# Electron-Labs/eth-lc-plonky2

Hardware: AMD Instinct MI355X
Metric: lc_proofs_per_hour (higher is better)
Workload: dtype u64

## Files before the change

### eth-lc-plonky2_amd/csrc/witness_rows.hip

```cpp
#include <cstring>
#include "internal.hpp"
#include "row_stage.hpp"
#include "sha_layout.hpp"
#include "sha_rows.hpp"
#include "pos_rows.hpp"
#include "prover_kernels.hpp"
#include "u32_rows.hpp"
#include "rec_rows.hpp"
#include "pos_plan.hpp"
#include "u32_plan.hpp"

using namespace lcp2;

namespace lcp2 {
int scratch_ensure(lcp2_ctx *ctx, int slot, size_t bytes, void **out) {
  if (ctx->scratch_bytes[slot] < bytes) {
    if (ctx->scratch[slot]) { LCP2_HIP(ctx, hipStreamSynchronize(ctx->stream)); LCP2_HIP(ctx, hipFree(ctx->scratch[slot])); ctx->scratch[slot] = nullptr; ctx->scratch_bytes[slot] = 0; }
    const size_t want = bytes + bytes / 4 + 4096;
    LCP2_HIP(ctx, hipMalloc(&ctx->scratch[slot], want));
    ctx->scratch_bytes[slot] = want;
  }
  *out = ctx->scratch[slot];
  return LCP2_OK;
}
}

namespace {
constexpr size_t ENDS_OK = ~(size_t)0;
size_t ends_problem(const uint32_t *ends, size_t count, size_t total) {
  if (!total) return ENDS_OK;
  for (size_t l = 0; l < count; l++)
    if (ends[l] < (l ? ends[l - 1] : 0) || ends[l] > total) return l;
  return count && ends[count - 1] == total ? ENDS_OK : count;
}
}

static_assert(sizeof(lcp2_sha_job) == sizeof(ShaJobDev) && sizeof(lcp2_cell) == sizeof(CellDev), "ABI structs must match the kernels'");

extern "C" int lcp2_sha256_witness(lcp2_ctx *ctx, const lcp2_sha_job *jobs, size_t njobs, const uint32_t *level_start, uint32_t nlevels,
                                   const uint32_t *words_in, size_t nwords, uint64_t *wires, uint64_t n, uint32_t *digests) {
  if (!ctx || !wires || (njobs && (!jobs || !level_start || nlevels == 0)) || (nwords && !words_in)) return LCP2_E_INVALID;
  if (njobs == 0) return LCP2_OK;
  if (const ShaProblem refused = sha_jobs_problem((const ShaJobDev *)jobs, njobs, level_start, nlevels, nwords, n); refused.problem)
    return ctx->fail(LCP2_E_INVALID, sha_problem_str(refused.problem));
  LCP2_HIP(ctx, hipSetDevice(ctx->device));
  void *d_jobs, *d_words, *d_rec;
  LCP2_TRY(scratch_ensure(ctx, 0, njobs * sizeof(lcp2_sha_job), &d_jobs));
  LCP2_TRY(scratch_ensure(ctx, 1, std::max<size_t>(nwords, 1) * 4, &d_words));
  LCP2_TRY(scratch_ensure(ctx, 2, njobs * (size_t)SHA_REC_WORDS * 4, &d_rec));
  Stage stage{ctx};
  LCP2_TRY(stage.behind(d_jobs, jobs, njobs * sizeof(lcp2_sha_job)));
  if (nwords) LCP2_TRY(stage.behind(d_words, words_in, nwords * 4));
  {
    ProfScope ps(ctx, LCP2_K_SHA256, 96.0 * njobs + 8.0 * 108 * SHA_ROWS * njobs);
    for (uint32_t l = 0; l < nlevels; l++)
      launch_sha_jobs_level(ctx->stream, (const ShaJobDev *)d_jobs, level_start[l], level_start[l + 1] - level_start[l],
                            (const uint32_t *)d_words, (uint32_t *)d_rec);
    launch_sha_fill_rows(ctx->stream, (const ShaJobDev *)d_jobs, (u32)njobs, (const uint32_t *)d_rec, (u64 *)wires, n);
  }
  LCP2_HIP(ctx, hipGetLastError());
  char *back = digests ? stage.room(njobs * 32) : nullptr;
  if (digests)
    LCP2_HIP(ctx, hipMemcpy2DAsync(back ? (void *)back : (void *)digests, 32, (const uint32_t *)d_rec + SHA_REC_DIGEST,
                                   (size_t)SHA_REC_WORDS * 4, 32, njobs, hipMemcpyDeviceToHost, ctx->stream));
  LCP2_HIP(ctx, hipStreamSynchronize(ctx->stream));
  if (back) memcpy(digests, back, njobs * 32);
  return LCP2_OK;
}

extern "C" int lcp2_scatter_cells(lcp2_ctx *ctx, const lcp2_cell *cells, size_t ncells, uint64_t *wires, uint64_t n) {
  if (!ctx || !wires || (ncells && !cells)) return LCP2_E_INVALID;
  if (!ncells) return LCP2_OK;
  if (scatter_cells_problem((const CellDev *)cells, ncells, n) != ncells) return ctx->fail(LCP2_E_INVALID, "scatter: row out of range");
  LCP2_HIP(ctx, hipSetDevice(ctx->device));
  void *d;
  LCP2_TRY(scratch_ensure(ctx, 3, ncells * sizeof(lcp2_cell), &d));
  LCP2_TRY(Stage{ctx}.behind(d, cells, ncells * sizeof(lcp2_cell)));
  launch_scatter_cells(ctx->stream, (const CellDev *)d, ncells, (u64 *)wires, n);
  LCP2_HIP(ctx, hipGetLastError());
  LCP2_HIP(ctx, hipStreamSynchronize(ctx->stream));
  return LCP2_OK;
}

extern "C" int lcp2_poseidon_gate_rows(lcp2_ctx *ctx, const lcp2_poseidon_row *rows, size_t nrows, uint64_t *wires, uint64_t n) {
  static_assert(sizeof(lcp2_poseidon_row) == sizeof(PoseidonRowDev), "row job layouts must agree");
  if (!ctx || !wires || (nrows && !rows)) return LCP2_E_INVALID;
  if (!nrows) return LCP2_OK;
  for (size_t i = 0; i < nrows; i++)
    if (pos_row_problem(((const PoseidonRowDev *)rows)[i], n)) return ctx->fail(LCP2_E_INVALID, "poseidon rows: row out of range or swap flag not boolean");
  LCP2_HIP(ctx, hipSetDevice(ctx->device));
  void *d;
  LCP2_TRY(scratch_ensure(ctx, 0, nrows * sizeof(lcp2_poseidon_row), &d));
  LCP2_TRY(Stage{ctx}.behind(d, rows, nrows * sizeof(lcp2_poseidon_row)));
  launch_poseidon_gate_rows(ctx->stream, (const PoseidonRowDev *)d, nrows, (u64 *)wires, n, ctx->d_rc);
  LCP2_HIP(ctx, hipGetLastError());
  LCP2_HIP(ctx, hipStreamSynchronize(ctx->stream));
  return LCP2_OK;
}

extern "C" int lcp2_u32_gate_rows(lcp2_ctx *ctx, const lcp2_u32_job *jobs, size_t njobs, lcp2_mem jobs_mem, uint64_t *wires, uint64_t n) {
  static_assert(sizeof(lcp2_u32_job) == 24 && sizeof(lcp2_u32_job) == sizeof(U32JobDev), "job layouts must agree");
  static_assert(LCP2_U32_ARITHMETIC == U32_KIND_ARITHMETIC && LCP2_U32_ADD_MANY == U32_KIND_ADD_MANY && LCP2_U32_SUBTRACTION == U32_KIND_SUBTRACTION &&
                LCP2_U32_RANGE_CHECK == U32_KIND_RANGE_CHECK && LCP2_U32_COMPARISON == U32_KIND_COMPARISON, "kind numbering must agree");
  if (!ctx || !wires || (njobs && !jobs)) return LCP2_E_INVALID;
  if (jobs_mem != LCP2_MEM_HOST && jobs_mem != LCP2_MEM_DEVICE) return ctx->fail(LCP2_E_INVALID, "u32 rows: bad lcp2_mem");
  if (!njobs) return LCP2_OK;
  const U32JobDev *list = (const U32JobDev *)jobs;
  if (jobs_mem == LCP2_MEM_HOST)
    for (size_t i = 0; i < njobs; i++)
      if (u32 problem = u32_job_problem(list[i], n))
        return ctx->fail(LCP2_E_INVALID, "u32 rows: job " + std::to_string(i) + ": " + u32_problem_str(problem));
  LCP2_HIP(ctx, hipSetDevice(ctx->device));
  RefusalFlag flag{ctx};
  LCP2_TRY(flag.begin());
  if (jobs_mem == LCP2_MEM_DEVICE) {
    launch_u32_gate_rows(ctx->stream, list, njobs, (u64 *)wires, n, flag.d);
  } else {
    constexpr size_t PIECE = (size_t)1 << 20;
    void *d;
    LCP2_TRY(scratch_ensure(ctx, 0, std::min(njobs, PIECE) * sizeof(lcp2_u32_job), &d));
    for (size_t at = 0; at < njobs; at += PIECE) {
      const size_t count = std::min(PIECE, njobs - at);
      LCP2_TRY(Stage{ctx}.behind(d, list + at, count * sizeof(lcp2_u32_job), njobs <= PIECE));
      launch_u32_gate_rows(ctx->stream, (const U32JobDev *)d, count, (u64 *)wires, n, flag.d);
    }
  }
  return flag.end("u32 rows", u32_problem_str, "the valid jobs are written");
}

namespace {
// ... 121 lines not shown
```

### eth-lc-plonky2_amd/host/builder.cpp

```cpp
#include <cstdio>
#include <algorithm>
#include <atomic>
#include <chrono>
#include <cstdlib>
#include <map>
#include <thread>
#include "host_internal.hpp"

namespace lc {

const uint32_t SHA_K[64] = {
    0x428a2f98, 0x71374491, 0xb5c0fbcf, 0xe9b5dba5, 0x3956c25b, 0x59f111f1, 0x923f82a4, 0xab1c5ed5, 0xd807aa98, 0x12835b01,
    0x243185be, 0x550c7dc3, 0x72be5d74, 0x80deb1fe, 0x9bdc06a7, 0xc19bf174, 0xe49b69c1, 0xefbe4786, 0x0fc19dc6, 0x240ca1cc,
    0x2de92c6f, 0x4a7484aa, 0x5cb0a9dc, 0x76f988da, 0x983e5152, 0xa831c66d, 0xb00327c8, 0xbf597fc7, 0xc6e00bf3, 0xd5a79147,
    0x06ca6351, 0x14292967, 0x27b70a85, 0x2e1b2138, 0x4d2c6dfc, 0x53380d13, 0x650a7354, 0x766a0abb, 0x81c2c92e, 0x92722c85,
    0xa2bfe8a1, 0xa81a664b, 0xc24b8b70, 0xc76c51a3, 0xd192e819, 0xd6990624, 0xf40e3585, 0x106aa070, 0x19a4c116, 0x1e376c08,
    0x2748774c, 0x34b0bcb5, 0x391c0cb3, 0x4ed8aa4a, 0x5b9cca4f, 0x682e6ff3, 0x748f82ee, 0x78a5636f, 0x84c87814, 0x8cc70208,
    0x90befffa, 0xa4506ceb, 0xbef9a3f7, 0xc67178f2};
const uint32_t SHA_IV[8] = {0x6a09e667, 0xbb67ae85, 0x3c6ef372, 0xa54ff53a, 0x510e527f, 0x9b05688c, 0x1f83d9ab, 0x5be0cd19};

static inline uint32_t rotr(uint32_t x, int r) { return (x >> r) | (x << (32 - r)); }

void PartialWitness::set_target(Target t, F value) { entries_.push_back({t.id, value % GOLDILOCKS_P}); }
void PartialWitness::set_hash256_target(const Hash256Target &t, const uint8_t v[32]) {
// ... 550 lines not shown
    case Op::SHA: break;
  }
}

void CircuitData::generate_witness(const PartialWitness &pw, std::vector<uint64_t> &wires, std::vector<F> &public_inputs) const {
  const Impl *d = impl_.get();
  const uint64_t n = 1ull << desc_.params.degree_bits;
  wires.assign((size_t)desc_.params.num_wires * n, 0);
  Values V(d);
  for (auto &e : pw.entries()) V.set(e.first, e.second, "PartialWitness");
  std::vector<lcp2_cell> raw;
  std::vector<const Op *> pending;
  for (const Op &op : d->ops) pending.push_back(&op);
  while (!pending.empty()) {
    std::vector<const Op *> waiting;
    for (const Op *opp : pending) {
      const Op &op = *opp;
      if (!host_op_ready(op, V)) { waiting.push_back(opp); continue; }
      if (op.kind == Op::SHA) eval_sha(op, V, wires, n);
      else host_op_eval(op, V, raw);
    }
    if (waiting.size() == pending.size()) throw UnsatisfiedError("a generator is waiting for a target that is never set");
    pending.swap(waiting);
  }
  for (const lcp2_cell &c : raw) wires[(size_t)c.col * n + c.row] = c.value;
  for (const CellBinding &c : d->cells) wires[(size_t)c.col * n + c.row] = V.get(c.var, "wire cell");
  public_inputs.clear();
  for (uint32_t v : d->public_inputs) public_inputs.push_back(V.get(v, "public input"));
}

CircuitData::~CircuitData() {
  if (impl_) {
    if (impl_->cell_buf_pinned) lcp2_host_unregister(impl_->ctx, impl_->cell_buf.data());
    if (impl_->d_wires) lcp2_buffer_free(impl_->ctx, impl_->d_wires);
    if (impl_->gpu) lcp2_circuit_destroy(impl_->gpu);
    if (impl_->verifier) lcp2_circuit_destroy(impl_->verifier);
  }
}

void CircuitData::verifier_only_data(uint64_t digest[4], std::vector<uint64_t> &cap) const {
  if (!impl_->gpu) throw std::runtime_error("verifier_only_data needs attach_gpu()");
  cap.assign((size_t)4 << desc_.params.cap_height, 0);
  if (lcp2_circuit_digest(impl_->gpu, digest, cap.data()) != LCP2_OK) throw std::runtime_error("lcp2_circuit_digest failed");
}

void CircuitData::attach_gpu(lcp2_ctx *ctx) {
  lcp2_circuit_desc cd = desc_.c_desc();
  int rc;
  if (impl_->compact) {
    lcp2_circuit_rows rows{};
    rows.gate_of_row = impl_->gate_of_row.data(); rows.num_rows = impl_->nrows; rows.pad_gate = G_NOOP;
    rows.row_constants = impl_->compact_consts.data();
    rows.bindings = impl_->compact_bindings.data(); rows.num_bindings = impl_->compact_bindings.size(); rows.bindings_mem = LCP2_MEM_HOST;
    rows.num_classes = (uint32_t)impl_->parent.size();
    cd.constants_sigmas = nullptr;
    rc = lcp2_circuit_create_from_rows(ctx, &cd, &rows, &impl_->gpu);
  } else {
    rc = lcp2_circuit_create(ctx, &cd, &impl_->gpu);
  }
  if (rc != LCP2_OK) throw std::runtime_error(std::string("lcp2_circuit_create: ") + lcp2_status_str(rc) + " (" + lcp2_last_error(ctx) + ")");
  impl_->ctx = ctx;
  const size_t bytes = (size_t)desc_.params.num_wires * ((size_t)1 << desc_.params.degree_bits) * 8;
  if (lcp2_buffer_alloc(ctx, bytes, &impl_->d_wires) != LCP2_OK || lcp2_buffer_zero(ctx, impl_->d_wires, bytes) != LCP2_OK)
    throw std::runtime_error(std::string("witness buffer: ") + lcp2_last_error(ctx));
}

// ... 77 lines not shown
          if (backoff < 8) backoff++;
          continue;
        }
        idle.fetch_add(1, std::memory_order_acq_rel);
        while (!stop.load(std::memory_order_acquire) && epoch.load(std::memory_order_acquire) == e0) {
          if (idle.load(std::memory_order_acquire) >= active.load(std::memory_order_acquire)) stop.store(true, std::memory_order_release);
          else std::this_thread::yield();
        }
        idle.fetch_sub(1, std::memory_order_acq_rel);
      }
    } catch (...) {
      failure[k] = std::current_exception();
      stop.store(true, std::memory_order_release);
    }
    active.fetch_sub(1, std::memory_order_acq_rel);
  };
  std::vector<std::thread> threads;
  for (unsigned k = 1; k < K; k++) threads.emplace_back(lane_main, k);
  lane_main(0);
  for (auto &t : threads) t.join();
  for (unsigned k = 0; k < K; k++) if (failure[k]) std::rethrow_exception(failure[k]);
  host_ops.clear();
  for (unsigned k = 0; k < K; k++) {
    host_ops.insert(host_ops.end(), mine[k].begin(), mine[k].end());
    cells.insert(cells.end(), lane_cells[k].begin(), lane_cells[k].end());
    pos_rows.insert(pos_rows.end(), lane_rows[k].begin(), lane_rows[k].end());
  }
  std::sort(host_ops.begin(), host_ops.end());
}

void CircuitData::generate_witness_gpu(const PartialWitness &pw, std::vector<F> &public_inputs) {
  Impl *d = impl_.get();
  if (!d->gpu) throw std::runtime_error("generate_witness_gpu needs attach_gpu()");
  const uint64_t n = 1ull << desc_.params.degree_bits;
  Values V(d);
  for (auto &e : pw.entries()) V.set(e.first, e.second, "PartialWitness");
  std::vector<const Op *> host_ops, sha_ops;
  for (const Op &op : d->ops) (op.kind == Op::SHA ? sha_ops : host_ops).push_back(&op);
  std::vector<lcp2_cell> cells;
  std::vector<lcp2_poseidon_row> pos_rows;
  const bool prof = getenv("LCP2_PROF") != nullptr;
  auto now = [] { return std::chrono::steady_clock::now(); };
  auto ms = [](std::chrono::steady_clock::time_point a, std::chrono::steady_clock::time_point b) { return std::chrono::duration<double, std::milli>(b - a).count(); };
  double t_host = 0;
  if (d->host_lanes.lane_of_op.size() != d->ops.size()) {
    unsigned want = 1;
    if (const char *e = getenv("LCP2_HOST_LANES")) want = (unsigned)atoi(e);
    d->host_lanes = plan_host_lanes(d, std::max(1u, std::min(want, 8u)));
  }
  HostPhaseStats st;
  bool recording = !d->gpu_plan.ready;
  GpuWitnessPlan recorded;
  size_t n_batches = 0;
  const auto t_begin = now();
  while (true) {
    const auto t0 = now();
    run_host_phase(d, d->host_lanes, host_ops, V, cells, pos_rows, st);
    t_host += ms(t0, now());
    if (sha_ops.empty()) break;
    const size_t batch_no = n_batches++;
    if (d->gpu_plan.ready && batch_no < d->gpu_plan.batches.size()) {
      const ShaBatchPlan &B = d->gpu_plan.batches[batch_no];
      bool applies = B.ops_left.size() < sha_ops.size();
      std::vector<uint32_t> words(B.word_vars.size());
      for (size_t k = 0; k < words.size() && applies; k++) {
        if (!V.known(B.word_vars[k])) applies = false;
        else words[k] = as_u32(V.val[B.word_vars[k]], "sha256 message word");
      }
      if (applies) {
        std::vector<uint32_t> digests(B.jobs.size() * 8);
        int rc = lcp2_sha256_witness(d->ctx, B.jobs.data(), B.jobs.size(), B.level_start.data(), (uint32_t)B.level_start.size() - 1, words.data(), words.size(),
                                     (uint64_t *)d->d_wires, n, digests.data());
        if (rc != LCP2_OK) throw std::runtime_error(std::string("lcp2_sha256_witness: ") + lcp2_status_str(rc) + " (" + lcp2_last_error(d->ctx) + ")");
        for (size_t k = 0; k < B.jobs.size(); k++)
          for (int w = 0; w < 8; w++) V.set(B.out[k][w], digests[k * 8 + w], "sha256 digest");
        sha_ops.clear();
        for (uint32_t k : B.ops_left) sha_ops.push_back(&d->ops[k]);
        continue;
      }
      d->gpu_plan = GpuWitnessPlan();
      recording = false;
    }
    std::map<uint32_t, uint32_t> produced;
    std::vector<lcp2_sha_job> jobs;
    std::vector<uint32_t> level, words, word_vars;
    std::vector<const Op *> batch, later;
    for (const Op *op : sha_ops) {
      lcp2_sha_job job{};
      job.first_row = op->first_row;
      uint32_t lvl = 0;
      bool ok = true;
      size_t words_mark = words.size();
      for (int i = 0; i < 16 && ok; i++) {
// ... 17 lines not shown
    for (uint32_t l : level) level_start[l + 1]++;
    for (uint32_t l = 0; l < nlev; l++) level_start[l + 1] += level_start[l];
    {
      std::vector<uint32_t> fill(level_start.begin(), level_start.end() - 1);
      for (uint32_t s = 0; s < jobs.size(); s++) { newslot[s] = fill[level[s]]++; order[newslot[s]] = s; }
    }
    std::vector<lcp2_sha_job> sorted(jobs.size());
    for (uint32_t s = 0; s < jobs.size(); s++) {
      lcp2_sha_job j = jobs[s];
      for (int i = 0; i < 16; i++)
        if (j.in_src[i] < 0) { uint32_t ref = (uint32_t)~j.in_src[i]; j.in_src[i] = ~(int32_t)(newslot[ref >> 3] * 8 + (ref & 7)); }
      sorted[newslot[s]] = j;
    }
    std::vector<uint32_t> digests(jobs.size() * 8);
    int rc = lcp2_sha256_witness(d->ctx, sorted.data(), sorted.size(), level_start.data(), nlev, words.data(), words.size(),
                                 (uint64_t *)d->d_wires, n, digests.data());
    if (rc != LCP2_OK) throw std::runtime_error(std::string("lcp2_sha256_witness: ") + lcp2_status_str(rc) + " (" + lcp2_last_error(d->ctx) + ")");
    for (uint32_t s = 0; s < batch.size(); s++)
      for (int w = 0; w < 8; w++) V.set(batch[s]->out8[w], digests[(size_t)newslot[s] * 8 + w], "sha256 digest");
    if (recording) {
      ShaBatchPlan B;
      B.jobs = sorted; B.word_vars = word_vars; B.level_start = level_start;
      for (const Op *op : later) B.ops_left.push_back((uint32_t)(op - d->ops.data()));
      B.out.resize(jobs.size());
      for (uint32_t s = 0; s < batch.size(); s++)
        for (int w = 0; w < 8; w++) B.out[newslot[s]][w] = d->find(batch[s]->out8[w]);
      recorded.batches.push_back(std::move(B));
    }
    sha_ops.swap(later);
  }
  if (!host_ops.empty()) throw UnsatisfiedError("a generator is waiting for a target that is never set");
  const auto t_rows = now();
  int rc = lcp2_poseidon_gate_rows(d->ctx, pos_rows.data(), pos_rows.size(), (uint64_t *)d->d_wires, n);
  if (rc != LCP2_OK) throw std::runtime_error(std::string("lcp2_poseidon_gate_rows: ") + lcp2_status_str(rc) + " (" + lcp2_last_error(d->ctx) + ")");
  if (!d->gpu_plan.ready) {
    GpuWitnessPlan fresh;
    std::vector<bool> listed(d->fill_copies ? d->parent.size() : 0, false);
    for (const CellBinding &c : d->cells) {
      uint32_t g = d->gate_of_row[c.row];
      if (g == G_SHA_ADD || g == G_SHA_ROUND_A || g == G_SHA_ROUND_E || g == G_SHA_SCHED || g == G_POSEIDON) continue;
      const uint32_t root = d->find(c.var);
      if (d->fill_copies) {
        if (listed[root]) continue;
        listed[root] = true;
      }
      fresh.host_cells.push_back(CellBinding{c.row, c.col, root});
    }
    if (recording) { fresh.batches = std::move(recorded.batches); fresh.ready = true; }
    d->gpu_plan = std::move(fresh);
  }
  std::vector<lcp2_cell> &buf = d->cell_buf;
  if (buf.size() != d->gpu_plan.host_cells.size()) {
    if (d->cell_buf_pinned) { lcp2_host_unregister(d->ctx, buf.data()); d->cell_buf_pinned = false; }
    buf.resize(d->gpu_plan.host_cells.size());
    for (size_t k = 0; k < buf.size(); k++) { buf[k].row = d->gpu_plan.host_cells[k].row; buf[k].col = d->gpu_plan.host_cells[k].col; }
    if (!buf.empty()) d->cell_buf_pinned = lcp2_host_register(d->ctx, buf.data(), buf.size() * sizeof(lcp2_cell)) == LCP2_OK;
  }
  for (size_t k = 0; k < buf.size(); k++) {
    const uint32_t var = d->gpu_plan.host_cells[k].var;
    if (!V.known(var)) throw UnsatisfiedError("target has no value: wire cell");
    buf[k].value = V.val[var];
  }
  const auto t_scatter = now();
  d->cells_sent = buf.size() + cells.size();
  if (d->fill_copies) {
    rc = lcp2_witness_fill_copies(d->gpu, buf.data(), buf.size(), LCP2_MEM_HOST, (uint64_t *)d->d_wires, nullptr);
    if (rc == LCP2_OK) rc = lcp2_witness_fill_copies(d->gpu, cells.data(), cells.size(), LCP2_MEM_HOST, (uint64_t *)d->d_wires, nullptr);
    if (rc != LCP2_OK) throw std::runtime_error(std::string("lcp2_witness_fill_copies: ") + lcp2_status_str(rc) + " (" + lcp2_last_error(d->ctx) + ")");
  } else {
    rc = lcp2_scatter_cells(d->ctx, buf.data(), buf.size(), (uint64_t *)d->d_wires, n);
    if (rc == LCP2_OK) rc = lcp2_scatter_cells(d->ctx, cells.data(), cells.size(), (uint64_t *)d->d_wires, n);
    if (rc != LCP2_OK) throw std::runtime_error(std::string("lcp2_scatter_cells: ") + lcp2_status_str(rc));
  }
  if (prof)
    printf("  witness generation %.2f ms: host generators %.2f ms on %u lane(s) (%zu sweeps, %zu visits of %zu ops, %zu PoseidonGate rows), SHA-256 batches %.2f ms, "
           "PoseidonGate rows on the device + cell list %.2f ms, scatter of %zu cells %.2f ms\n",
           ms(t_begin, now()), t_host, d->host_lanes.lanes, st.sweeps, st.visits, d->ops.size(), pos_rows.size(), ms(t_begin, t_rows) - t_host, ms(t_rows, t_scatter), cells.size() + buf.size(), ms(t_scatter, now()));
  public_inputs.clear();
  for (uint32_t v : d->public_inputs) public_inputs.push_back(V.get(v, "public input"));
}

void CircuitData::set_fill_copies(bool on) {
  if (impl_->fill_copies == on) return;
  impl_->fill_copies = on;
  impl_->gpu_plan = GpuWitnessPlan();
}
size_t CircuitData::cells_sent_last() const { return impl_->cells_sent; }

void CircuitData::read_device_witness(std::vector<uint64_t> &wires) const {
  const size_t words = (size_t)desc_.params.num_wires << desc_.params.degree_bits;
  wires.resize(words);
  if (!impl_->d_wires || lcp2_buffer_read(impl_->ctx, wires.data(), impl_->d_wires, words * 8) != LCP2_OK)
    throw std::runtime_error("read_device_witness failed");
}

ProofWithPublicInputs CircuitData::prove(const PartialWitness &pw) {
  if (!impl_->gpu) throw std::runtime_error("CircuitData::prove needs attach_gpu(): there is no CPU prover in this library");
  ProofWithPublicInputs out;
  generate_witness_gpu(pw, out.public_inputs);
  out.proof.assign(lcp2_proof_words(&desc_.params), 0);
  int rc = lcp2_prove(impl_->gpu, (const uint64_t *)impl_->d_wires, LCP2_MEM_DEVICE, out.public_inputs.data(), out.public_inputs.size(),
                      out.proof.data(), out.proof.size());
  if (rc == LCP2_E_UNSAT) throw UnsatisfiedError(std::string("lcp2_prove: ") + lcp2_last_error(impl_->ctx));
  if (rc != LCP2_OK) throw std::runtime_error(std::string("lcp2_prove: ") + lcp2_status_str(rc) + " (" + lcp2_last_error(impl_->ctx) + ")");
  return out;
}

std::string CircuitData::describe_report(const lcp2_witness_report &r) const {
  if (r.gate_violations == 0 && r.copy_violations == 0) return "the witness satisfies every gate and copy constraint";
  auto cell = [](uint64_t row, uint32_t wire) { return "(" + std::to_string(row) + ", " + std::to_string(wire) + ")"; };
  std::string text;
  if (r.gate_violations) {
    const char *name = r.gate_index < desc_.gates.size() && r.gate_index < G_COUNT ? gate_name(r.gate_index) : "gate ?";
    text = "row " + std::to_string(r.gate_row) + ", gate " + name + ", constraint " + std::to_string(r.gate_constraint) + " (" +
           std::to_string(r.gate_violations) + " gate constraints violated)";
  }
  if (r.copy_violations) {
    if (!text.empty()) text += "; ";
    text += "copy constraint " + cell(r.copy_row, r.copy_wire) + " != " +
            (r.copy_to_wire == 0xFFFFFFFFu ? std::string("(no cell: the sigma value is no cell id)") : cell(r.copy_to_row, r.copy_to_wire)) + " (" +
// ... 66 lines not shown
```

### eth-lc-plonky2_amd/host/host_internal.hpp

```cpp
#pragma once
#include <algorithm>
#include <cstring>
#include <functional>
#include "lc_plonky2.hpp"
#include "../csrc/pos_rows.hpp"

namespace lc {

constexpr int SHA_ADD_OPS = 3;
constexpr uint32_t ARITH_OPS = 20;
constexpr uint32_t SHA_ROWS_PER_HASH = 48 + 128 + 3 + 128 + 3;

struct GateSetLayout {
  std::vector<std::pair<uint32_t, uint32_t>> groups;
  uint32_t num_selectors = 0, num_regs = 1;
  std::vector<lcp2_gate> gates;
  std::vector<uint32_t> code;
  std::vector<uint64_t> imm;
};
GateSetLayout build_gate_set(uint32_t max_degree);

using lcp2::POS_WIRE_INPUT; using lcp2::POS_WIRE_OUTPUT; using lcp2::POS_WIRE_SWAP; using lcp2::POS_WIRE_DELTA; using lcp2::POS_WIRE_PARTIAL;
using lcp2::POS_GATE_WIRES; using lcp2::pos_wire_full_sbox_0; using lcp2::pos_wire_full_sbox_1;
const uint64_t *poseidon_round_constants();
// ... 18 lines not shown

extern const uint32_t SHA_K[64];
extern const uint32_t SHA_IV[8];

struct Op {
  enum Kind { CONST, ARITH, SHA, BITS, POSEIDON, INV, EXT_INV, SPLIT32, HINT } kind;
  uint32_t out = 0, x = 0, y = 0, z = 0;
  F c0 = 0, c1 = 0;
  std::array<uint32_t, 16> in{};
  std::array<uint32_t, 8> out8{};
  uint32_t first_row = 0;
  std::vector<uint32_t> hint_in;
  std::function<void(const std::vector<F> &, std::vector<F> &)> hint_fn;
  std::vector<uint32_t> internal;
};

struct CellBinding { uint32_t row, col, var; };
struct HostLanes {
  std::vector<uint8_t> lane_of_op;
  unsigned lanes = 1;
};

struct ShaBatchPlan {
  std::vector<lcp2_sha_job> jobs;
  std::vector<uint32_t> word_vars;
  std::vector<uint32_t> level_start;
  std::vector<std::array<uint32_t, 8>> out;
  std::vector<uint32_t> ops_left;
};
struct GpuWitnessPlan {
  bool ready = false;
  std::vector<ShaBatchPlan> batches;
  std::vector<CellBinding> host_cells;
};

struct CircuitData::Impl {
  CircuitConfig config;
  uint32_t nrows = 0;
  std::vector<uint32_t> gate_of_row;
  std::vector<std::array<F, 2>> row_consts;
  std::vector<CellBinding> cells;
  std::vector<uint32_t> parent;
  std::vector<Op> ops;
  std::vector<uint32_t> public_inputs;
  lcp2_ctx *ctx = nullptr;
  void *d_wires = nullptr;
  lcp2_circuit *gpu = nullptr;
  lcp2_circuit *verifier = nullptr;
  HostLanes host_lanes;
  GpuWitnessPlan gpu_plan;
  std::vector<lcp2_cell> cell_buf;
  bool cell_buf_pinned = false;
  bool compact = false;
  std::vector<uint64_t> compact_consts;
  std::vector<lcp2_copy_binding> compact_bindings;
  std::vector<std::pair<uint32_t, uint32_t>> selector_groups;
  BuildTimes times;
  bool fill_copies = false;
  size_t cells_sent = 0;
  mutable std::vector<F> value_store;
  mutable std::vector<uint32_t> stamp_store;
  mutable uint32_t epoch = 0;
  uint32_t find(uint32_t v) const { while (parent[v] != v) v = parent[v]; return v; }
};

void expand_constants_sigmas(const CircuitData::Impl *d, CircuitDescription &D, BuildTimes *times);

}
```

### eth-lc-plonky2_amd/host/lc_plonky2.hpp

```cpp
#pragma once
#include <array>
#include <cstdint>
#include <functional>
#include <map>
#include <memory>
#include <stdexcept>
#include <string>
#include <vector>
#include "../../include/lcp2.h"

namespace lc {

using F = uint64_t;
constexpr F GOLDILOCKS_P = 0xFFFFFFFF00000001ull;

struct Target { uint32_t id = 0xFFFFFFFFu; };
struct BoolTarget { Target target; };
struct U32Target { Target t; };
using Hash256Target = std::array<U32Target, 8>;

struct UnsatisfiedError : std::runtime_error { using std::runtime_error::runtime_error; };
struct VerifyError : std::runtime_error { using std::runtime_error::runtime_error; };

struct CircuitConfig {
// ... 88 lines not shown
};

struct BuildTimes { double gadgets_ms = 0, matrix_ms = 0, identity_ms = 0, classes_ms = 0, cycles_ms = 0; };

struct CircuitDescription {
  lcp2_params params{};
  std::vector<uint64_t> constants_sigmas;
  std::vector<uint64_t> k_is;
  uint32_t num_selectors = 0;
  std::vector<lcp2_gate> gates;
  std::vector<uint32_t> code;
  std::vector<uint64_t> imm;
  uint32_t num_public_inputs = 0, num_regs = 1;
  lcp2_circuit_desc c_desc() const;
};

class CircuitData {
 public:
  ~CircuitData();
  const CircuitDescription &description() const { return desc_; }
  const CircuitDescription &expanded_description() const;
  BuildTimes build_times() const;
  size_t build_upload_bytes() const;
  uint32_t degree_bits() const { return desc_.params.degree_bits; }
  uint32_t quotient_degree_factor() const { return desc_.params.quotient_degree_factor; }
  void generate_witness(const PartialWitness &pw, std::vector<uint64_t> &wires, std::vector<F> &public_inputs) const;
  void attach_gpu(lcp2_ctx *ctx);
  void verifier_only_data(uint64_t digest[4], std::vector<uint64_t> &constants_sigmas_cap) const;
  ProofWithPublicInputs prove(const PartialWitness &pw);
  void generate_witness_gpu(const PartialWitness &pw, std::vector<F> &public_inputs);
  void read_device_witness(std::vector<uint64_t> &wires) const;
  void set_fill_copies(bool on);
  size_t cells_sent_last() const;
  std::string diagnose(const PartialWitness &pw);
  std::string diagnose_witness(const std::vector<uint64_t> &wires, const std::vector<F> &public_inputs) const;
  std::string describe_report(const lcp2_witness_report &report) const;
  void verify(const ProofWithPublicInputs &proof) const;
  bool verify_batch(const uint64_t *proofs, size_t count, const uint64_t *public_inputs, int32_t *failed_checks) const;
  struct Impl;
  const Impl *impl_for_tools() const { return impl_.get(); }

 private:
  friend class CircuitBuilder;
  CircuitData() = default;
  mutable CircuitDescription desc_;
  std::unique_ptr<Impl> impl_;
};

}
```

### include/lcp2.h

```cpp
#ifndef LCP2_H
#define LCP2_H
#include <stddef.h>
#include <stdint.h>

#ifdef __cplusplus
extern "C" {
#endif

#define LCP2_ABI_VERSION 2

typedef enum {
  LCP2_OK = 0,
  LCP2_E_INVALID = -1,
  LCP2_E_NODEVICE = -2,
  LCP2_E_HIP = -3,
  LCP2_E_OOM = -4,
  LCP2_E_UNSAT = -5,
  LCP2_E_UNSUPPORTED = -6,
  LCP2_E_VERIFY = -7
} lcp2_status;

typedef enum { LCP2_MEM_HOST = 0, LCP2_MEM_DEVICE = 1 } lcp2_mem;

#define LCP2_MAX_FRI_LAYERS 8
// ... 46 lines not shown
  LCP2_FIELD_SHL = 16
};
int lcp2_field_op_batch(lcp2_ctx *ctx, const uint64_t *a, const uint64_t *b, uint64_t *out, size_t count, uint32_t op, lcp2_mem mem);

int lcp2_merkle_cap(lcp2_ctx *ctx, const uint64_t *leaves, size_t nleaves, size_t leaf_len,
                    uint32_t cap_height, lcp2_mem mem, uint64_t *cap );

int lcp2_ntt_batch(lcp2_ctx *ctx, uint64_t *data, size_t ncols, uint32_t log_n, int inverse,
                   uint64_t shift, lcp2_mem mem);

int lcp2_lde_batch(lcp2_ctx *ctx, const uint64_t *coeffs, uint64_t *out, size_t ncols, uint32_t log_n,
                   uint32_t rate_bits, lcp2_mem mem);

int lcp2_sha256_tree(lcp2_ctx *ctx, const uint8_t *leaves, uint32_t height, size_t trees,
                     uint8_t *nodes, uint32_t *round_trace, lcp2_mem mem);

typedef struct {
  uint32_t first_row;
  int32_t in_src[16];
} lcp2_sha_job;
typedef struct {
  uint32_t row, col;
  uint64_t value;
} lcp2_cell;
int lcp2_sha256_witness(lcp2_ctx *ctx, const lcp2_sha_job *jobs, size_t njobs, const uint32_t *level_start, uint32_t nlevels,
                        const uint32_t *words_in, size_t nwords, uint64_t *wires, uint64_t n, uint32_t *digests);
int lcp2_scatter_cells(lcp2_ctx *ctx, const lcp2_cell *cells, size_t ncells, uint64_t *wires, uint64_t n);
typedef struct {
  uint32_t row;
  uint32_t swap;
  uint64_t in[12];
} lcp2_poseidon_row;
int lcp2_poseidon_gate_rows(lcp2_ctx *ctx, const lcp2_poseidon_row *rows, size_t nrows, uint64_t *wires, uint64_t n);
enum { LCP2_U32_ARITHMETIC = 0, LCP2_U32_ADD_MANY = 1, LCP2_U32_SUBTRACTION = 2, LCP2_U32_RANGE_CHECK = 3, LCP2_U32_COMPARISON = 4 };
typedef struct {
  uint32_t row;
  uint16_t kind;
  uint16_t op;
  uint32_t in[4];
} lcp2_u32_job;
int lcp2_u32_gate_rows(lcp2_ctx *ctx, const lcp2_u32_job *jobs, size_t njobs, lcp2_mem jobs_mem,
                       uint64_t *wires , uint64_t n);

enum { LCP2_REC_ARITHMETIC = 0, LCP2_REC_BASE_SUM, LCP2_REC_ARITHMETIC_EXT, LCP2_REC_MUL_EXT, LCP2_REC_REDUCING,
       LCP2_REC_REDUCING_EXT, LCP2_REC_POSEIDON_MDS, LCP2_REC_RANDOM_ACCESS, LCP2_REC_EXPONENTIATION,
       LCP2_REC_COSET_INTERPOLATION, LCP2_REC_KINDS };
enum { LCP2_REC_IMM = 0, LCP2_REC_CELL = 1 };
typedef struct {
  uint64_t v;
  uint32_t col;
  uint32_t src;
} lcp2_rec_operand;
typedef struct {
  uint32_t row;
  uint16_t kind;
  uint16_t op;
  uint32_t first_operand, reserved;
} lcp2_rec_job;
int lcp2_rec_gate_rows(lcp2_ctx *ctx, const lcp2_rec_job *jobs, size_t njobs,
                       const lcp2_rec_operand *operands, size_t noperands,
                       const uint32_t *level_ends , size_t nlevels,
                       lcp2_mem lists_mem ,
                       uint64_t *wires , uint32_t ncols, uint64_t n);

enum { LCP2_PLAN_IMM = 0, LCP2_PLAN_CELL = 1, LCP2_PLAN_PREV = 2 };
typedef struct { uint32_t row, first_operand; } lcp2_pos_job;
// ... 224 lines not shown
```

Before: 9196.

## Replay recorded witness plan with async enqueues and a single stream wait

Adds non-blocking enqueue variants of the SHA-256, Poseidon-row and scatter entry points, and a replay path for witness generation once a single-batch plan has been recorded. The replay launches the SHA-256 kernels before running the host generators, so host work overlaps device work, then enqueues the rows and cells and waits on the stream only once. Digest-dependent generators and late cells are handled afterwards. Pinned host buffers for words and digests let the copies run asynchronously. The risk is added complexity and a fallback to the recording path whenever replay preconditions fail.

```diff
diff --git a/eth-lc-plonky2_amd/csrc/witness_rows.hip b/eth-lc-plonky2_amd/csrc/witness_rows.hip
--- a/eth-lc-plonky2_amd/csrc/witness_rows.hip
+++ b/eth-lc-plonky2_amd/csrc/witness_rows.hip
@@ -37,8 +37,9 @@
 
 static_assert(sizeof(lcp2_sha_job) == sizeof(ShaJobDev) && sizeof(lcp2_cell) == sizeof(CellDev), "ABI structs must match the kernels'");
 
-extern "C" int lcp2_sha256_witness(lcp2_ctx *ctx, const lcp2_sha_job *jobs, size_t njobs, const uint32_t *level_start, uint32_t nlevels,
-                                   const uint32_t *words_in, size_t nwords, uint64_t *wires, uint64_t n, uint32_t *digests) {
+namespace {
+int sha256_witness(lcp2_ctx *ctx, const lcp2_sha_job *jobs, size_t njobs, const uint32_t *level_start, uint32_t nlevels,
+                   const uint32_t *words_in, size_t nwords, uint64_t *wires, uint64_t n, uint32_t *digests, bool wait) {
   if (!ctx || !wires || (njobs && (!jobs || !level_start || nlevels == 0)) || (nwords && !words_in)) return LCP2_E_INVALID;
   if (njobs == 0) return LCP2_OK;
   if (const ShaProblem refused = sha_jobs_problem((const ShaJobDev *)jobs, njobs, level_start, nlevels, nwords, n); refused.problem)
@@ -49,8 +50,8 @@
   LCP2_TRY(scratch_ensure(ctx, 1, std::max<size_t>(nwords, 1) * 4, &d_words));
   LCP2_TRY(scratch_ensure(ctx, 2, njobs * (size_t)SHA_REC_WORDS * 4, &d_rec));
   Stage stage{ctx};
-  LCP2_TRY(stage.behind(d_jobs, jobs, njobs * sizeof(lcp2_sha_job)));
-  if (nwords) LCP2_TRY(stage.behind(d_words, words_in, nwords * 4));
+  LCP2_TRY(stage.behind(d_jobs, jobs, njobs * sizeof(lcp2_sha_job), wait));
+  if (nwords) LCP2_TRY(stage.behind(d_words, words_in, nwords * 4, wait));
   {
     ProfScope ps(ctx, LCP2_K_SHA256, 96.0 * njobs + 8.0 * 108 * SHA_ROWS * njobs);
     for (uint32_t l = 0; l < nlevels; l++)
@@ -59,30 +60,31 @@
     launch_sha_fill_rows(ctx->stream, (const ShaJobDev *)d_jobs, (u32)njobs, (const uint32_t *)d_rec, (u64 *)wires, n);
   }
   LCP2_HIP(ctx, hipGetLastError());
-  char *back = digests ? stage.room(njobs * 32) : nullptr;
+  char *back = digests && wait ? stage.room(njobs * 32) : nullptr;
   if (digests)
     LCP2_HIP(ctx, hipMemcpy2DAsync(back ? (void *)back : (void *)digests, 32, (const uint32_t *)d_rec + SHA_REC_DIGEST,
                                    (size_t)SHA_REC_WORDS * 4, 32, njobs, hipMemcpyDeviceToHost, ctx->stream));
+  if (!wait) return LCP2_OK;
   LCP2_HIP(ctx, hipStreamSynchronize(ctx->stream));
   if (back) memcpy(digests, back, njobs * 32);
   return LCP2_OK;
 }
 
-extern "C" int lcp2_scatter_cells(lcp2_ctx *ctx, const lcp2_cell *cells, size_t ncells, uint64_t *wires, uint64_t n) {
+int scatter_cells(lcp2_ctx *ctx, const lcp2_cell *cells, size_t ncells, uint64_t *wires, uint64_t n, bool wait) {
   if (!ctx || !wires || (ncells && !cells)) return LCP2_E_INVALID;
   if (!ncells) return LCP2_OK;
   if (scatter_cells_problem((const CellDev *)cells, ncells, n) != ncells) return ctx->fail(LCP2_E_INVALID, "scatter: row out of range");
   LCP2_HIP(ctx, hipSetDevice(ctx->device));
   void *d;
   LCP2_TRY(scratch_ensure(ctx, 3, ncells * sizeof(lcp2_cell), &d));
-  LCP2_TRY(Stage{ctx}.behind(d, cells, ncells * sizeof(lcp2_cell)));
+  LCP2_TRY(Stage{ctx}.behind(d, cells, ncells * sizeof(lcp2_cell), wait));
   launch_scatter_cells(ctx->stream, (const CellDev *)d, ncells, (u64 *)wires, n);
   LCP2_HIP(ctx, hipGetLastError());
-  LCP2_HIP(ctx, hipStreamSynchronize(ctx->stream));
-  return LCP2_OK;
-}
-
-extern "C" int lcp2_poseidon_gate_rows(lcp2_ctx *ctx, const lcp2_poseidon_row *rows, size_t nrows, uint64_t *wires, uint64_t n) {
+  if (wait) LCP2_HIP(ctx, hipStreamSynchronize(ctx->stream));
+  return LCP2_OK;
+}
+
+int poseidon_gate_rows(lcp2_ctx *ctx, const lcp2_poseidon_row *rows, size_t nrows, uint64_t *wires, uint64_t n, bool wait) {
   static_assert(sizeof(lcp2_poseidon_row) == sizeof(PoseidonRowDev), "row job layouts must agree");
   if (!ctx || !wires || (nrows && !rows)) return LCP2_E_INVALID;
   if (!nrows) return LCP2_OK;
@@ -91,11 +93,33 @@
   LCP2_HIP(ctx, hipSetDevice(ctx->device));
   void *d;
   LCP2_TRY(scratch_ensure(ctx, 0, nrows * sizeof(lcp2_poseidon_row), &d));
-  LCP2_TRY(Stage{ctx}.behind(d, rows, nrows * sizeof(lcp2_poseidon_row)));
+  LCP2_TRY(Stage{ctx}.behind(d, rows, nrows * sizeof(lcp2_poseidon_row), wait));
   launch_poseidon_gate_rows(ctx->stream, (const PoseidonRowDev *)d, nrows, (u64 *)wires, n, ctx->d_rc);
   LCP2_HIP(ctx, hipGetLastError());
-  LCP2_HIP(ctx, hipStreamSynchronize(ctx->stream));
-  return LCP2_OK;
+  if (wait) LCP2_HIP(ctx, hipStreamSynchronize(ctx->stream));
+  return LCP2_OK;
+}
+}
+
+extern "C" int lcp2_sha256_witness(lcp2_ctx *ctx, const lcp2_sha_job *jobs, size_t njobs, const uint32_t *level_start, uint32_t nlevels,
+                                   const uint32_t *words_in, size_t nwords, uint64_t *wires, uint64_t n, uint32_t *digests) {
+  return sha256_witness(ctx, jobs, njobs, level_start, nlevels, words_in, nwords, wires, n, digests, true);
+}
+extern "C" int lcp2_scatter_cells(lcp2_ctx *ctx, const lcp2_cell *cells, size_t ncells, uint64_t *wires, uint64_t n) {
+  return scatter_cells(ctx, cells, ncells, wires, n, true);
+}
+extern "C" int lcp2_poseidon_gate_rows(lcp2_ctx *ctx, const lcp2_poseidon_row *rows, size_t nrows, uint64_t *wires, uint64_t n) {
+  return poseidon_gate_rows(ctx, rows, nrows, wires, n, true);
+}
+extern "C" int lcp2_sha256_witness_enqueue(lcp2_ctx *ctx, const lcp2_sha_job *jobs, size_t njobs, const uint32_t *level_start, uint32_t nlevels,
+                                           const uint32_t *words_in, size_t nwords, uint64_t *wires, uint64_t n, uint32_t *digests) {
+  return sha256_witness(ctx, jobs, njobs, level_start, nlevels, words_in, nwords, wires, n, digests, false);
+}
+extern "C" int lcp2_scatter_cells_enqueue(lcp2_ctx *ctx, const lcp2_cell *cells, size_t ncells, uint64_t *wires, uint64_t n) {
+  return scatter_cells(ctx, cells, ncells, wires, n, false);
+}
+extern "C" int lcp2_poseidon_gate_rows_enqueue(lcp2_ctx *ctx, const lcp2_poseidon_row *rows, size_t nrows, uint64_t *wires, uint64_t n) {
+  return poseidon_gate_rows(ctx, rows, nrows, wires, n, false);
 }
 
 extern "C" int lcp2_u32_gate_rows(lcp2_ctx *ctx, const lcp2_u32_job *jobs, size_t njobs, lcp2_mem jobs_mem, uint64_t *wires, uint64_t n) {
diff --git a/eth-lc-plonky2_amd/host/builder.cpp b/eth-lc-plonky2_amd/host/builder.cpp
--- a/eth-lc-plonky2_amd/host/builder.cpp
+++ b/eth-lc-plonky2_amd/host/builder.cpp
@@ -606,6 +606,8 @@
 CircuitData::~CircuitData() {
   if (impl_) {
     if (impl_->cell_buf_pinned) lcp2_host_unregister(impl_->ctx, impl_->cell_buf.data());
+    impl_->replay_words.release(impl_->ctx);
+    impl_->replay_digests.release(impl_->ctx);
     if (impl_->d_wires) lcp2_buffer_free(impl_->ctx, impl_->d_wires);
     if (impl_->gpu) lcp2_circuit_destroy(impl_->gpu);
     if (impl_->verifier) lcp2_circuit_destroy(impl_->verifier);
@@ -749,6 +751,16 @@
 void CircuitData::generate_witness_gpu(const PartialWitness &pw, std::vector<F> &public_inputs) {
   Impl *d = impl_.get();
   if (!d->gpu) throw std::runtime_error("generate_witness_gpu needs attach_gpu()");
+  const char *sw = getenv("LCP2_WITNESS_REPLAY");
+  if (d->gpu_plan.ready && d->gpu_plan.replayable && !d->fill_copies && !(sw && sw[0] == '0' && !sw[1])) {
+    if (replay_witness(pw, public_inputs)) return;
+    d->gpu_plan = GpuWitnessPlan();
+  }
+  generate_witness_recording(pw, public_inputs);
+}
+
+void CircuitData::generate_witness_recording(const PartialWitness &pw, std::vector<F> &public_inputs) {
+  Impl *d = impl_.get();
   const uint64_t n = 1ull << desc_.params.degree_bits;
   Values V(d);
   for (auto &e : pw.entries()) V.set(e.first, e.second, "PartialWitness");
@@ -768,14 +780,17 @@
   HostPhaseStats st;
   bool recording = !d->gpu_plan.ready;
   GpuWitnessPlan recorded;
-  size_t n_batches = 0;
+  size_t n_batches = 0, rows_first = 0;
+  uint32_t syncs = 0, late_ops = 0;
   const auto t_begin = now();
   while (true) {
     const auto t0 = now();
     run_host_phase(d, d->host_lanes, host_ops, V, cells, pos_rows, st);
     t_host += ms(t0, now());
+    if (n_batches == 0) { late_ops = (uint32_t)host_ops.size(); rows_first = pos_rows.size(); }
     if (sha_ops.empty()) break;
     const size_t batch_no = n_batches++;
+    syncs++;
     if (d->gpu_plan.ready && batch_no < d->gpu_plan.batches.size()) {
       const ShaBatchPlan &B = d->gpu_plan.batches[batch_no];
       bool applies = B.ops_left.size() < sha_ops.size();
@@ -859,8 +874,10 @@
   if (!host_ops.empty()) throw UnsatisfiedError("a generator is waiting for a target that is never set");
   const auto t_rows = now();
   int rc = lcp2_poseidon_gate_rows(d->ctx, pos_rows.data(), pos_rows.size(), (uint64_t *)d->d_wires, n);
+  syncs += !pos_rows.empty();
   if (rc != LCP2_OK) throw std::runtime_error(std::string("lcp2_poseidon_gate_rows: ") + lcp2_status_str(rc) + " (" + lcp2_last_error(d->ctx) + ")");
-  if (!d->gpu_plan.ready) {
+  const bool plans = !d->gpu_plan.ready;
+  if (plans) {
     GpuWitnessPlan fresh;
     std::vector<bool> listed(d->fill_copies ? d->parent.size() : 0, false);
     for (const CellBinding &c : d->cells) {
@@ -873,7 +890,7 @@
       }
       fresh.host_cells.push_back(CellBinding{c.row, c.col, root});
     }
-    if (recording) { fresh.batches = std::move(recorded.batches); fresh.ready = true; }
+    if (recording) { fresh.batches = std::move(recorded.batches); fresh.ready = true; fresh.replayable = fresh.batches.size() == 1; }
     d->gpu_plan = std::move(fresh);
   }
   std::vector<lcp2_cell> &buf = d->cell_buf;
@@ -890,6 +907,9 @@
   }
   const auto t_scatter = now();
   d->cells_sent = buf.size() + cells.size();
+  syncs += (uint32_t)!buf.empty() + (uint32_t)!cells.empty();
+  d->waits_last = syncs;
+  if (plans) { d->gpu_plan.syncs = syncs; d->gpu_plan.late_ops = late_ops; d->gpu_plan.late_rows = (uint32_t)(pos_rows.size() - rows_first); }
   if (d->fill_copies) {
     rc = lcp2_witness_fill_copies(d->gpu, buf.data(), buf.size(), LCP2_MEM_HOST, (uint64_t *)d->d_wires, nullptr);
     if (rc == LCP2_OK) rc = lcp2_witness_fill_copies(d->gpu, cells.data(), cells.size(), LCP2_MEM_HOST, (uint64_t *)d->d_wires, nullptr);
@@ -899,6 +919,14 @@
     if (rc == LCP2_OK) rc = lcp2_scatter_cells(d->ctx, cells.data(), cells.size(), (uint64_t *)d->d_wires, n);
     if (rc != LCP2_OK) throw std::runtime_error(std::string("lcp2_scatter_cells: ") + lcp2_status_str(rc));
   }
+  if (prof) {
+    const GpuWitnessPlan &P = d->gpu_plan;
+    printf("  witness round trips: %zu SHA-256 batch(es), %u waits for the stream, %u host generators and %zu PoseidonGate rows behind a digest; %s\n",
+           n_batches, syncs, late_ops, pos_rows.size() - rows_first,
+           !P.ready ? "no plan recorded" : P.replayable ? "the record replays with one wait"
+                                                        : n_batches > 1 ? "not replayable: host generators between the batches make message words, every batch boundary stays"
+                                                                        : "not replayable: no SHA-256 batch");
+  }
   if (prof)
     printf("  witness generation %.2f ms: host generators %.2f ms on %u lane(s) (%zu sweeps, %zu visits of %zu ops, %zu PoseidonGate rows), SHA-256 batches %.2f ms, "
            "PoseidonGate rows on the device + cell list %.2f ms, scatter of %zu cells %.2f ms\n",
@@ -907,12 +935,120 @@
   for (uint32_t v : d->public_inputs) public_inputs.push_back(V.get(v, "public input"));
 }
 
+bool CircuitData::replay_witness(const PartialWitness &pw, std::vector<F> &public_inputs) {
+  Impl *d = impl_.get();
+  const uint64_t n = 1ull << desc_.params.degree_bits;
+  GpuWitnessPlan &P = d->gpu_plan;
+  const ShaBatchPlan &B = P.batches[0];
+  const bool prof = getenv("LCP2_PROF") != nullptr;
+  auto now = [] { return std::chrono::steady_clock::now(); };
+  auto ms = [](std::chrono::steady_clock::time_point a, std::chrono::steady_clock::time_point b) { return std::chrono::duration<double, std::milli>(b - a).count(); };
+  const auto t_begin = now();
+  bool in_flight = false;
+  auto hip = [&](int rc, const char *what) {
+    if (rc != LCP2_OK) throw std::runtime_error(std::string(what) + ": " + lcp2_status_str(rc) + " (" + lcp2_last_error(d->ctx) + ")");
+  };
+  try {
+    Values V(d);
+    for (auto &e : pw.entries()) V.set(e.first, e.second, "PartialWitness");
+    std::vector<const Op *> host_ops;
+    for (const Op &op : d->ops) {
+      if (op.kind == Op::CONST) V.set(op.out, op.c0, "constant");
+      else if (op.kind != Op::SHA) host_ops.push_back(&op);
+    }
+    d->replay_words.size_to(d->ctx, B.word_vars.size());
+    d->replay_digests.size_to(d->ctx, B.jobs.size() * 8);
+    uint32_t *words = d->replay_words.v.data(), *digests = d->replay_digests.v.data();
+    auto fetch_words = [&] {
+      for (size_t k = 0; k < B.word_vars.size(); k++) {
+        if (!V.known(B.word_vars[k])) return false;
+        words[k] = as_u32(V.val[B.word_vars[k]], "sha256 message word");
+      }
+      return true;
+    };
+    auto enqueue_sha = [&] {
+      in_flight = true;
+      hip(lcp2_sha256_witness_enqueue(d->ctx, B.jobs.data(), B.jobs.size(), B.level_start.data(), (uint32_t)B.level_start.size() - 1, words, B.word_vars.size(),
+                                      (uint64_t *)d->d_wires, n, digests), "lcp2_sha256_witness_enqueue");
+    };
+    std::vector<lcp2_poseidon_row> &rows = d->replay_rows;
+    std::vector<lcp2_cell> &raw = d->replay_raw;
+    rows.clear(); raw.clear();
+    HostPhaseStats st;
+    const bool words_first = fetch_words();
+    if (words_first) enqueue_sha();
+    const auto t_sha = now();
+    run_host_phase(d, d->host_lanes, host_ops, V, raw, rows, st);
+    const auto t_host = now();
+    if (!words_first) {
+      if (!fetch_words()) return false;
+      enqueue_sha();
+    }
+    in_flight = true;
+    hip(lcp2_poseidon_gate_rows_enqueue(d->ctx, rows.data(), rows.size(), (uint64_t *)d->d_wires, n), "lcp2_poseidon_gate_rows_enqueue");
+    std::vector<lcp2_cell> &buf = d->cell_buf;
+    if (buf.size() != P.host_cells.size()) return lcp2_ctx_sync(d->ctx), false;
+    std::vector<uint32_t> late;
+    for (size_t k = 0; k < buf.size(); k++) {
+      const uint32_t var = P.host_cells[k].var;
+      if (V.known(var)) buf[k].value = V.val[var];
+      else late.push_back((uint32_t)k);
+    }
+    hip(lcp2_scatter_cells_enqueue(d->ctx, buf.data(), buf.size(), (uint64_t *)d->d_wires, n), "lcp2_scatter_cells_enqueue");
+    hip(lcp2_scatter_cells_enqueue(d->ctx, raw.data(), raw.size(), (uint64_t *)d->d_wires, n), "lcp2_scatter_cells_enqueue");
+    const auto t_wait = now();
+    hip(lcp2_ctx_sync(d->ctx), "lcp2_ctx_sync");
+    in_flight = false;
+    const auto t_digests = now();
+    for (size_t k = 0; k < B.jobs.size(); k++)
+      for (int w = 0; w < 8; w++) V.set(B.out[k][w], digests[k * 8 + w], "sha256 digest");
+    uint32_t waits = 1;
+    const size_t late_ops = host_ops.size();
+    size_t late_rows = 0, late_raw = 0;
+    if (!host_ops.empty() || !late.empty()) {
+      std::vector<lcp2_poseidon_row> rows2;
+      std::vector<lcp2_cell> cells2;
+      run_host_phase(d, d->host_lanes, host_ops, V, cells2, rows2, st);
+      if (!host_ops.empty()) throw UnsatisfiedError("a generator is waiting for a target that is never set");
+      late_rows = rows2.size();
+      late_raw = cells2.size();
+      for (uint32_t k : late) {
+        if (!V.known(P.host_cells[k].var)) throw UnsatisfiedError("target has no value: wire cell");
+        buf[k].value = V.val[P.host_cells[k].var];
+        cells2.push_back(buf[k]);
+      }
+      hip(lcp2_poseidon_gate_rows(d->ctx, rows2.data(), rows2.size(), (uint64_t *)d->d_wires, n), "lcp2_poseidon_gate_rows");
+      hip(lcp2_scatter_cells(d->ctx, cells2.data(), cells2.size(), (uint64_t *)d->d_wires, n), "lcp2_scatter_cells");
+      waits += (uint32_t)!rows2.empty() + (uint32_t)!cells2.empty();
+    }
+    P.late_cells = (uint32_t)late.size();
+    d->waits_last = waits;
+    d->cells_sent = buf.size() + raw.size() + late_raw;
+    public_inputs.clear();
+    for (uint32_t v : d->public_inputs) public_inputs.push_back(V.get(v, "public input"));
+    if (prof)
+      printf("  witness generation %.2f ms (replayed, %u wait(s) for the stream; recorded path: %u): words + SHA-256 enqueue %.2f ms (%s the host generators), host generators %.2f ms "
+             "(%zu sweeps, %zu visits of %zu ops, %zu PoseidonGate rows), rows + %zu cells enqueued %.2f ms, wait %.2f ms, digests and what is behind them %.2f ms "
+             "(%zu generators, %zu PoseidonGate rows, %zu cells)\n",
+             ms(t_begin, now()), waits, P.syncs, ms(t_begin, t_sha), words_first ? "before" : "after", ms(t_sha, t_host), st.sweeps, st.visits, d->ops.size(),
+             rows.size(), buf.size() + raw.size(), ms(t_host, t_wait), ms(t_wait, t_digests), ms(t_digests, now()), late_ops, late_rows, late.size());
+    return true;
+  } catch (const UnsatisfiedError &) {
+    if (in_flight) lcp2_ctx_sync(d->ctx);
+    return false;
+  } catch (...) {
+    if (in_flight) lcp2_ctx_sync(d->ctx);
+    throw;
+  }
+}
+
 void CircuitData::set_fill_copies(bool on) {
   if (impl_->fill_copies == on) return;
   impl_->fill_copies = on;
   impl_->gpu_plan = GpuWitnessPlan();
 }
 size_t CircuitData::cells_sent_last() const { return impl_->cells_sent; }
+size_t CircuitData::witness_waits_last() const { return impl_->waits_last; }
 
 void CircuitData::read_device_witness(std::vector<uint64_t> &wires) const {
   const size_t words = (size_t)desc_.params.num_wires << desc_.params.degree_bits;
diff --git a/eth-lc-plonky2_amd/host/host_internal.hpp b/eth-lc-plonky2_amd/host/host_internal.hpp
--- a/eth-lc-plonky2_amd/host/host_internal.hpp
+++ b/eth-lc-plonky2_amd/host/host_internal.hpp
@@ -74,6 +74,20 @@
   bool ready = false;
   std::vector<ShaBatchPlan> batches;
   std::vector<CellBinding> host_cells;
+  bool replayable = false;
+  uint32_t syncs = 0, late_ops = 0, late_rows = 0, late_cells = 0;
+};
+
+template <class T> struct PinnedBuffer {
+  std::vector<T> v;
+  bool pinned = false;
+  void release(lcp2_ctx *ctx) { if (pinned) { lcp2_host_unregister(ctx, v.data()); pinned = false; } }
+  void size_to(lcp2_ctx *ctx, size_t count) {
+    if (v.size() == count) return;
+    release(ctx);
+    v.assign(count, T{});
+    if (count) pinned = lcp2_host_register(ctx, v.data(), count * sizeof(T)) == LCP2_OK;
+  }
 };
 
 struct CircuitData::Impl {
@@ -93,6 +107,9 @@
   GpuWitnessPlan gpu_plan;
   std::vector<lcp2_cell> cell_buf;
   bool cell_buf_pinned = false;
+  PinnedBuffer<uint32_t> replay_words, replay_digests;
+  std::vector<lcp2_poseidon_row> replay_rows;
+  std::vector<lcp2_cell> replay_raw;
   bool compact = false;
   std::vector<uint64_t> compact_consts;
   std::vector<lcp2_copy_binding> compact_bindings;
@@ -100,6 +117,7 @@
   BuildTimes times;
   bool fill_copies = false;
   size_t cells_sent = 0;
+  size_t waits_last = 0;
   mutable std::vector<F> value_store;
   mutable std::vector<uint32_t> stamp_store;
   mutable uint32_t epoch = 0;
diff --git a/eth-lc-plonky2_amd/host/lc_plonky2.hpp b/eth-lc-plonky2_amd/host/lc_plonky2.hpp
--- a/eth-lc-plonky2_amd/host/lc_plonky2.hpp
+++ b/eth-lc-plonky2_amd/host/lc_plonky2.hpp
@@ -144,6 +144,7 @@
   void read_device_witness(std::vector<uint64_t> &wires) const;
   void set_fill_copies(bool on);
   size_t cells_sent_last() const;
+  size_t witness_waits_last() const;
   std::string diagnose(const PartialWitness &pw);
   std::string diagnose_witness(const std::vector<uint64_t> &wires, const std::vector<F> &public_inputs) const;
   std::string describe_report(const lcp2_witness_report &report) const;
@@ -155,6 +156,8 @@
  private:
   friend class CircuitBuilder;
   CircuitData() = default;
+  void generate_witness_recording(const PartialWitness &pw, std::vector<F> &public_inputs);
+  bool replay_witness(const PartialWitness &pw, std::vector<F> &public_inputs);
   mutable CircuitDescription desc_;
   std::unique_ptr<Impl> impl_;
 };
diff --git a/include/lcp2.h b/include/lcp2.h
--- a/include/lcp2.h
+++ b/include/lcp2.h
@@ -102,6 +102,10 @@
   uint64_t in[12];
 } lcp2_poseidon_row;
 int lcp2_poseidon_gate_rows(lcp2_ctx *ctx, const lcp2_poseidon_row *rows, size_t nrows, uint64_t *wires, uint64_t n);
+int lcp2_sha256_witness_enqueue(lcp2_ctx *ctx, const lcp2_sha_job *jobs, size_t njobs, const uint32_t *level_start, uint32_t nlevels,
+                                const uint32_t *words_in, size_t nwords, uint64_t *wires, uint64_t n, uint32_t *digests);
+int lcp2_scatter_cells_enqueue(lcp2_ctx *ctx, const lcp2_cell *cells, size_t ncells, uint64_t *wires, uint64_t n);
+int lcp2_poseidon_gate_rows_enqueue(lcp2_ctx *ctx, const lcp2_poseidon_row *rows, size_t nrows, uint64_t *wires, uint64_t n);
 enum { LCP2_U32_ARITHMETIC = 0, LCP2_U32_ADD_MANY = 1, LCP2_U32_SUBTRACTION = 2, LCP2_U32_RANGE_CHECK = 3, LCP2_U32_COMPARISON = 4 };
 typedef struct {
   uint32_t row;
```

Result: no change. 9213 (median of 6 runs) (+0.2%).
